# HerreraKrachTeichmann/NJODE

Measured on AMD Instinct MI355X. Metric: paths/sec (training step) on 20k Black-Scholes, 100 steps, higher is better.
Workload: dtype f32; 1 GPU; BlackScholes 20000 paths/GPU x 100 grid steps, every rank's paths as one batch, hidden_size=10, 3x(50,50) tanh nets, dropout 0.1, train step = plan+fwd+bwd+Adam; global_batch=20000, n_obs_rows=199470, euler_steps_per_batch=1820212, params=10071, parallelism=dp1

## Files before the change

njode_amd/csrc/njode_cfg.hip:

```cpp
#include <type_traits>

#include "njode_route.h"
#if NJ_PART >= 4
#include "njode_chain.h"
#include "njode_chain_seg.h"
#include "njode_chain_dw.h"
#endif

#define NJ_CAT_(a, b) a##b
#define NJ_CAT(a, b) NJ_CAT_(a, b)

namespace njode {

#ifndef NJ_RNN
#define NJ_RNN 0
#endif
using C = Cfg<NJ_D, NJ_H, NJ_DO, NJ_NH, NJ_W, NJ_ACT, (NJ_MASKED != 0), (NJ_CURT != 0),
              (NJ_RES != 0), (NJ_RNN != 0)>;

hipError_t NJ_CAT(njode_seg_forward_, NJ_ID)(const KArgs& a, const Route& r, hipStream_t st);
hipError_t NJ_CAT(njode_seg_backward_, NJ_ID)(const KArgs& a, const Route& r, hipStream_t st);
constexpr bool HAS_MFMA = C::NH == 2 && !C::MASKED && !C::RNN && C::DO <= 16 && C::W < 64;
constexpr bool HAS_MFMA_LOCK = C::NH == 2 && !C::RNN && C::W < 64 && C::H <= 64 && C::DO <= 64;
constexpr bool HAS_MFMA_SWEEP =
// ... 68 lines not shown
    }
    if constexpr (HAS_SPLIT) {
      const int nb = (int)gridDim.x - n_pack;
      drop_bits_tile_steps<C>(a, ((int)blockIdx.x - n_pack) * 4 + (threadIdx.x >> 6), nb * 4);
    }
  }
}

template <class CC> static void launch_pack_frags(const KArgs& a, hipStream_t st, bool bits = false) {
  if constexpr (HAS_MFMA) {
    using ES = typename EncS<CC>::type;
    using DS = typename DecS<CC>::type;
    const int n_pack = cdiv((2 * MF<CC>::NALL + ES::NALL + DS::NALL) * 64, 256);
    if (bits) {
      const long long work = a.seg_chain ? (long long)a.K * a.B / 64 + 1
                                         : (long long)cdiv(a.n_obs, 16) * cdiv(a.K > 0 ? a.K : 1, 8);
      const int nb = (int)(work / 4 + 1 < 1024 ? work / 4 + 1 : 1024);
      k_pack_all_bits<CC, ES, DS><<<n_pack + nb, 256, 0, st>>>(a, n_pack);
    } else {
      k_pack_all<CC, ES, DS><<<n_pack, 256, 0, st>>>(a.P, a.frag, a.frag2, a.frag_enc, a.frag_dec, a.dc.inv_keep,
                                                  a.plan_sync_zero);
    }
  }
}
template <class CC, bool DROP> static void launch_mfma_enc(const KArgs& a, const Route& r, hipStream_t st) {
  if constexpr (HAS_MFMA) {
    const int n_tiles = cdiv(a.n_obs + a.B, 16);
    k_encode_rows_mfma<CC, DROP><<<n_tiles < r.enc_blocks ? n_tiles : r.enc_blocks, 64, 0, st>>>(a);
  }
}
template <class CC> static void lock_pack_frags(const KArgs& a, hipStream_t st) {
  if constexpr (HAS_MFMA_LOCK) {
    using ES = typename EncS<CC>::type;
    using DS = typename DecS<CC>::type;
    k_pack_frags<CC><<<cdiv(MF<CC>::NALL * 64, 256), 256, 0, st>>>(a.P, a.frag);
    k_pack_net<typename CC::Enc, ES><<<cdiv(ES::NALL * 64, 256), 256, 0, st>>>(a.P + CC::OFF_ENC,
                                                                             a.frag_enc);
    k_pack_net<typename CC::Dec, DS><<<cdiv(DS::NALL * 64, 256), 256, 0, st>>>(a.P + CC::OFF_DEC,
                                                                             a.frag_dec);
  }
}
template <class CC, bool DROP> static void launch_mfma_jump(const KArgs& a, hipStream_t st) {
  if constexpr (HAS_MFMA) {
    const int n_tiles = cdiv(a.n_obs, 16);
    k_jump_rows_mfma<CC, DROP><<<n_tiles < 2048 ? n_tiles : 2048, 64, 0, st>>>(a);
  }
}
template <class CC, bool DROP> static void launch_ode_bwd_mfma(const KArgs& a, const Route& r, hipStream_t st) {
  if constexpr (HAS_MFMA) {
    if constexpr (HAS_SPLIT) {
      if (r.ode_split) {
        ProfScope ps("k_ode_bwd_mixed", st);
        if (r.tile_q_on) k_ode_bwd_mixed<CC, DROP, true><<<a.n_blocks_bwd, 256, 0, st>>>(a);
        else k_ode_bwd_mixed<CC, DROP, false><<<a.n_blocks_bwd, 256, 0, st>>>(a);
        return;
      }
    }
    ProfScope ps("k_ode_bwd_mfma", st);
    k_ode_bwd_mfma<CC, DROP><<<a.n_waves_ode / 4, 256, 0, st>>>(a);
  }
}
template <class CC, bool DROP> static void launch_jump_rows_bwd(const KArgs& a, hipStream_t st) {
  if constexpr (HAS_MFMA) {
    ProfScope ps("k_jump_rows_bwd_mfma", st);
    k_jump_rows_bwd_mfma<CC, DROP><<<a.n_waves_rows / 4, 256, 0, st>>>(a);
  }
}
template <class CC, bool DROP>
static void launch_mfma_rows_bwd(const KArgs& a, const Route& r, hipStream_t st) {
  if constexpr (HAS_MFMA) {
    if (r.defer_loss != 2) launch_jump_rows_bwd<CC, DROP>(a, st);
    if (r.seg_chain) NJ_CAT(njode_seg_chain_backward_, NJ_ID)(a, r, st);
    else launch_ode_bwd_mfma<CC, DROP>(a, r, st);
    if (!r.dw_enc_fused) {
      ProfScope ps("k_encode_rows_bwd_mfma", st);
      k_encode_rows_bwd_mfma<CC, DROP><<<a.n_waves_rows / 4, 256, 0, st>>>(a);
    }
  }
}
template <class CC, bool DROP, bool TAIL>
static void launch_mfma_fwd(const KArgs& a, const Route& r, hipStream_t st) {
  if constexpr (HAS_MFMA) {
    const int n_tiles = cdiv(TAIL ? a.B : a.n_obs, 16);
    if constexpr (HAS_SPLIT) {
      if (r.ode_split) {
        if constexpr (TAIL) {
          k_ode_fwd_split<CC, DROP, true><<<n_tiles < 1024 ? n_tiles : 1024, 256, 0, st>>>(a);
        }
        else if (a.plan_job) {
          const PlanJob job = *(const PlanJob*)a.plan_job;
          k_ode_fwd_mixed_plan<CC, DROP, false><<<a.n_blocks_fwd + job.P, 256, 0, st>>>(a, job);
        }
        else if (r.enc_fused) k_ode_fwd_mixed<CC, DROP, true><<<a.n_blocks_fwd, 256, 0, st>>>(a);
        else k_ode_fwd_mixed<CC, DROP, false><<<a.n_blocks_fwd, 256, 0, st>>>(a);
        return;
      }
    }
    k_ode_fwd_mfma<CC, DROP, TAIL><<<n_tiles < 4096 ? n_tiles : 4096, 64, 0, st>>>(a);
  }
}

hipError_t NJ_CAT(njode_lock_forward_, NJ_ID)(const KArgs& a, const Route& r, hipStream_t st);
hipError_t NJ_CAT(njode_lock_backward_, NJ_ID)(const KArgs& a, const Route& r, hipStream_t st);

#if NJ_PART == 0
template <bool DROP, bool TAIL, int ODE> static void launch_ode_fwd(const KArgs& a, const Route& r, hipStream_t st) {
// ... 348 lines not shown
```

njode_amd/csrc/njode_kernels.h:

```cpp
#pragma once
#include "njode_device.h"

namespace njode {

constexpr uint32_t NET_ODE = 0, NET_ENC = 1, NET_DEC = 2, NET_DEC_BJ = 3, NET_DEC_ROW = 4;
constexpr uint32_t TKEY_START = 0xffffffffu;

template <int D_, int H_, int DO_, int NH_, int W_, int ACT_, bool MASKED_, bool CURT_,
          bool RES_, bool RNN_ = false>
struct Cfg {
  static constexpr int D = D_, H = H_, DO = DO_, NH = NH_, W = (NH_ > 0 ? W_ : 1), ACT = ACT_;
  static constexpr bool MASKED = MASKED_, CURT = CURT_, RES = RES_, RNN = RNN_;
  static constexpr int ODE_IN = D + H + (CURT ? 3 : 2);
  static constexpr int ENC_IN = MASKED ? 2 * D : D;
  using Ode = NetL<ODE_IN, H, NH, W_>;
  using Enc = NetL<ENC_IN, H, NH, W_>;
  using Dec = NetL<H, DO, NH, W_>;
  static constexpr int OFF_ODE = 0, OFF_ENC = Ode::SIZE, OFF_DEC = Ode::SIZE + Enc::SIZE;
  static constexpr int OFF_GRU = OFF_DEC + Dec::SIZE;
  static constexpr int G_WIH = 0, G_WHH = 3 * H * D, G_BIH = G_WHH + 3 * H * H, G_BHH = G_BIH + 3 * H;
  static constexpr int GRU_SIZE = G_BHH + 3 * H;
  static constexpr int P = OFF_GRU + (RNN ? GRU_SIZE : 0);
  static_assert(!(RNN && MASKED), "the GRU jump is not defined for masked models");
  static constexpr int ENC_CASE = !RES ? 0 : (D <= H ? 1 : 2);
// ... 294 lines not shown
      r = a.order[jj];
      b = a.obs_idx[r];
      n = valid ? a.item_len[r] : 0;
      kbeg = a.item_kbeg[r];
      prev = a.item_prev[r];
    }
    const int pv = prev >= 0 ? prev : 0;
    const float tprev = a.n_obs > 0 ? a.time_f32[a.t_of_row[pv]] : 0.0f;
    tau = prev >= 0 ? tprev : 0.0f;
    const float* xp = prev >= 0 ? a.X + (size_t)pv * C::D : a.start_X + (size_t)b * C::D;
#pragma unroll
    for (int i = 0; i < C::D; ++i) tx[i] = tanh_f(xp[i]);
  }
  NJ_DEV const float* h0(const KArgs& a) const {
    return prev >= 0 ? a.h0row + (size_t)prev * C::H : a.h0start + (size_t)b * C::H;
  }
  static constexpr int PACKF = 4 + 4 * ((1 + C::D + 3) / 4);
  NJ_DEV void store_pack(float* pack, int j) const {
    typedef float v4 __attribute__((ext_vector_type(4)));
    float* p = pack + (size_t)j * PACKF;
    const v4 head = {__int_as_float(r), __int_as_float(n), __int_as_float(kbeg), __int_as_float(b)};
    *(v4*)p = head;
#pragma unroll
    for (int q = 0; q < (PACKF - 4) / 4; ++q) {
      v4 v;
#pragma unroll
      for (int e = 0; e < 4; ++e) {
        const int i = 4 * q + e;
        v[e] = i == 0 ? tau : (i <= C::D ? tx[i - 1 < C::D ? (i > 0 ? i - 1 : 0) : 0] : 0.0f);
      }
      *(v4*)(p + 4 + 4 * q) = v;
    }
  }
  NJ_DEV void load_pack(const float* pack, int j, bool valid) {
    typedef float v4 __attribute__((ext_vector_type(4)));
    const float* p = pack + (size_t)j * PACKF;
    const v4 head = *(const v4*)p;
    r = __float_as_int(head[0]);
    n = valid ? __float_as_int(head[1]) : 0;
    kbeg = __float_as_int(head[2]);
    b = __float_as_int(head[3]);
    prev = -1;
#pragma unroll
    for (int q = 0; q < (PACKF - 4) / 4; ++q) {
      const v4 v = *(const v4*)(p + 4 + 4 * q);
#pragma unroll
      for (int e = 0; e < 4; ++e) {
        const int i = 4 * q + e;
        if (i == 0) tau = v[e];
        else if (i <= C::D) tx[i - 1 < C::D ? i - 1 : 0] = v[e];
      }
    }
  }
};

template <class C, bool DROP, bool TAIL, bool WLDS>
__global__ void __launch_bounds__(WLDS ? 256 : 64) k_ode_fwd_items(KArgs a) {
  const bool SAVE = !TAIL && a.save_traj != 0;
  constexpr int NT = WLDS ? 256 : 64;
  using NL = typename C::Ode;
  __shared__ __attribute__((aligned(16))) float wl[WLDS ? NL::SIZE : 4];
  if constexpr (WLDS) {
    for (int i = threadIdx.x; i < NL::SIZE; i += NT) wl[i] = a.P[C::OFF_ODE + i];
    __syncthreads();
  }
  const int n_items = TAIL ? a.B : a.n_obs;
  const int j = blockIdx.x * NT + threadIdx.x;
  const bool valid = j < n_items;
  Item<C> it;
  it.template load<TAIL>(a, j, valid);
  float h[C::H];
  load_vec(it.h0(a), h);
  const int nmax = wave_max(it.n);
  float* const trash = a.trash + threadIdx.x * C::H;
  for (int s = 0; s < nmax; ++s) {
    const bool active = s < it.n;
    const int k = active ? it.kbeg + s : 0;
    if (SAVE) {
      float* dst = active ? a.traj + (size_t)(a.base_s[s] + j) * C::H : trash;
      store_vec(dst, h);
    }
    const float dt = active ? a.step_dt[k] : 0.0f, t = a.step_t[k];
    float in0[C::ODE_IN], a1[C::W], a2[C::W], f[C::H];
    ode_input<C>(it.tx, h, it.tau, t, in0);
    Masks<C, DROP> mk;
    mk.draw(a, a.gid0 + it.b, (uint32_t)k, NET_ODE);
    if constexpr (WLDS)
      net_fwd<NL, C::ACT, DROP>((lcp)wl, in0, f, a1, a2, mk.m1, mk.m2, a.dc.inv_keep);
    else
      net_fwd<NL, C::ACT, DROP>(as_cfp(a.P) + C::OFF_ODE, in0, f, a1, a2, mk.m1, mk.m2,
                                a.dc.inv_keep);
#pragma unroll
    for (int i = 0; i < C::H; ++i) h[i] = fmaf(dt, f[i], h[i]);
  }
  float* out = TAIL ? a.hT + (size_t)it.b * C::H : a.h_end + (size_t)it.r * C::H;
  store_vec(valid ? out : trash, h);
}

template <class C, bool DROP>
__global__ void __launch_bounds__(64) k_jump_rows(KArgs a) {
  const int r = blockIdx.x * 64 + threadIdx.x;
  if (r >= a.n_obs) return;
  const int b = a.obs_idx[r];
  const uint32_t tkey = (uint32_t)a.k_jump[a.t_of_row[r]];
  const cfp Pd = as_cfp(a.P) + C::OFF_DEC;
  float h[C::H], th[C::H], a1[C::W], a2[C::W], y[C::DO], ybj[C::DO], x[C::D], mask[C::D];
// ... 318 lines not shown
```

njode_amd/csrc/njode_mfma_split.h:

```cpp
#pragma once
#include "njode_mfma.h"
#include "njode_ode2.h"
#include "njode_plan.h"

namespace njode {

template <class C, bool TWO = (C::NH == 2)> struct SplitOk { static constexpr bool value = false; };
template <class C> struct SplitOk<C, true> {
  static constexpr bool value = MF<C>::MT1 == 4 && MF<C>::MTH == 1 && !C::MASKED && !C::RNN;
};

constexpr int XROWS = 64;
constexpr int XFLOATS = XROWS * IMG_STRIDE;
constexpr int TROWS = 16;
constexpr int TFLOATS = TROWS * IMG_STRIDE;

template <class C, bool BWD> struct SplitFrags {
  using M = MF<C>;
  float A1[M::Q0], A2[M::Q1], A3[4];
  float B3[BWD ? M::QH : 1], B2[BWD ? M::QW : 1], B1[BWD ? 4 : 1];
  NJ_DEV void load(const float* frag, int w, int lane) {
#pragma unroll
    for (int q = 0; q < M::Q0; ++q) A1[q] = frag[(M::F1 + w * M::Q0 + q) * 64 + lane];
#pragma unroll
// ... 201 lines not shown
    s += PR[(3 * NQ + r) * 64 + lane];
    out[r] = s;
  }
}

template <class C> struct OdeFwdSplitLds { static constexpr int FLOATS = XFLOATS + 4 * MF<C>::QH * 64; };
template <class C, bool DROP, bool TAIL, bool SAVE>
NJ_DEV void ode_fwd_split(const KArgs& a, lfp lds_raw, int worker, int n_workers, int tile0, int tile1) {
  static_assert(!(TAIL && SAVE), "tail items are never checkpointed");
  using M = MF<C>;
  lfp X1 = lds_raw, PR = X1 + XFLOATS;
  const int lane = threadIdx.x & 63, g = lane >> 4, c = lane & 15;
  const int w = __builtin_amdgcn_readfirstlane(threadIdx.x >> 6);
  for (int i = threadIdx.x; i < XFLOATS; i += 256) lds_raw[i] = 0.0f;
  SplitFrags<C, false> F;
  F.load(a.frag, w, lane);
  In0Const<C> K0;
  K0.init(g);
  __syncthreads();
  const bool bits_ahead = DROP && !TAIL && a.dbits_ready != 0;

  const int n_items = TAIL ? a.B : a.n_obs;
  const int n_tiles = tile1 - tile0;
  float* const trash = a.trash + lane * C::H;
  for (int round = 0; round * n_workers < n_tiles; ++round) {
    const int rel = snake_tile(round, worker, n_workers);
    if (rel >= n_tiles) continue;
    const int tile = tile0 + rel;
    const int j = tile * 16 + c;
    const bool valid = j < n_items;
    Item<C> it;
    it.template load<TAIL>(a, j, valid);
    const float* h0 = it.h0(a);
    float h[M::QH];
#pragma unroll
    for (int q = 0; q < M::QH; ++q) {
      const int u = 4 * q + g;
      h[q] = u < C::H ? h0[u < C::H ? u : 0] : 0.0f;
    }
    const int nmax = uniform(wave_max(it.n));
    float dt_r = 0.0f, t_r = 0.0f;
    uint32_t kb_r = 0;
    long long b16_n = 0;
    if (nmax > 0) {
      const int k0 = it.n > 0 ? it.kbeg : 0;
      dt_r = a.step_dt[k0];
      t_r = a.step_t[k0];
      b16_n = (SAVE || bits_ahead) ? sload_ll(a.base16_s, 0) : 0;
      if (bits_ahead) kb_r = a.dbits[(size_t)(b16_n / 16 + tile) * 64 + lane];
    }
    if constexpr (SAVE) {
      if (a.item_pack) {
        if (w == 0 && g == 0) it.store_pack(a.item_pack, j);
        const long long bl = sload_ll(a.base16_s, nmax > 0 ? nmax - 1 : 0);
        if (threadIdx.x == 0) a.tile_last[tile] = bl;
      }
    }
    vm_drain();
    for (int s = 0; s < nmax; ++s) {
      const bool active = s < it.n;
      const int k = active ? it.kbeg + s : 0;
      const float dt = active ? dt_r : 0.0f, t = t_r;
      const uint32_t kb = kb_r;
      const long long b16 = b16_n;
      {
        const int sn = s + 1 < nmax ? s + 1 : s;
        const int kn = sn < it.n ? it.kbeg + sn : 0;
        dt_r = a.step_dt[kn];
        t_r = a.step_t[kn];
        if (SAVE || bits_ahead) b16_n = sload_ll(a.base16_s, sn);
        if (bits_ahead) kb_r = a.dbits[(size_t)(b16_n / 16 + tile) * 64 + lane];
      }
      float b0[M::Q0], a1l[4], a2l[4], a1u[4], a2u[4];
      in0_fill_c<C, 0>(b0, h, it.tx, it.tau, t - it.tau, g, K0);
      uint32_t k1 = 0, k2 = 0;
      if constexpr (DROP) {
        if (bits_ahead) {
          k1 = (kb >> (4 * w)) & 15u;
          k2 = (kb >> (16 + 4 * w)) & 15u;
        } else {
          split_keep_bits<C, DROP>(a, it.b, k, g, w, k1, k2);
        }
      }
      split_hidden_layers<C, DROP, false>(F, X1, b0, a1l, a2l, a1u, a2u, k1, k2, a.dc.inv_keep, g, c, w);
      if constexpr (SAVE) split_rec_store<C>(rec_block<C>(a.act, b16, tile), a.trash, lane, w, a1u, a2u, h);
      f32x4 part = {0.f, 0.f, 0.f, 0.f};
#pragma unroll
      for (int r = 0; r < 4; ++r)
        if (4 * w + r < M::Q1) part = mfma4(F.A3[r], a2l[r], part);
      float f[M::QH];
      split_reduce<M::QH>(PR, part, f, lane, w);
#pragma unroll
      for (int q = 0; q < M::QH; ++q) h[q] = fmaf(dt, f[q], h[q]);
    }
    if (w == 0) {
      float* out = valid ? (TAIL ? a.hT + (size_t)it.b * C::H : a.h_end + (size_t)it.r * C::H) : trash;
#pragma unroll
      for (int q = 0; q < M::QH; ++q) {
        const int u = 4 * q + g;
        float* dst = u < C::H ? out + u : trash;
        *dst = h[q];
      }
    }
  }
}

template <class C> struct OdeBwdSplitLds {
// ... 366 lines not shown
template <class C, bool DROP, bool TAIL>
__global__ void __launch_bounds__(256, 2) k_ode_fwd_split(KArgs a) {
  __shared__ __attribute__((aligned(16))) float lds_raw[OdeFwdSplitLds<C>::FLOATS];
  const int n_items = TAIL ? a.B : a.n_obs;
  ode_fwd_split<C, DROP, TAIL, false>(a, (lfp)lds_raw, blockIdx.x, gridDim.x, 0, (n_items + 15) / 16);
}

template <class C, bool ENC, bool PLAN> struct OdeFwdMixedLds {
  static constexpr int OWN = OdeFwdSplitLds<C>::FLOATS + (ENC ? EncFwdLds<C>::FLOATS : 0);
  static constexpr int FLOATS = (PLAN && PLAN_LDS_INTS > OWN) ? PLAN_LDS_INTS : OWN;
};
template <class C, bool DROP, bool ENC, bool PLAN>
__device__ __forceinline__ void ode_fwd_mixed_body(const KArgs& a, lfp lds_raw, int bid, int nblocks) {
  const int n_tiles = (a.n_obs + 15) / 16, ns = a.n_split_fwd;
  const int T = (int)a.base_s[a.K + 2];
  const bool save = a.save_traj != 0;
  if (save && bid == 0 && threadIdx.x == 0) { a.tile_q[0] = 0; a.tile_q[1] = 0; a.tile_q[2] = 0; }
  if (bid < ns) {
    if (save) ode_fwd_split<C, DROP, false, true>(a, lds_raw, bid, ns, 0, T);
    else ode_fwd_split<C, DROP, false, false>(a, lds_raw, bid, ns, 0, T);
  } else {
    const int wave = (bid - ns) * 4 + uniform(threadIdx.x >> 6);
    const int nw = (nblocks - ns) * 4;
    if constexpr (ENC) {
      lfp enc_img = lds_raw + OdeFwdSplitLds<C>::FLOATS;
      EncFwdLds<C>::stage(enc_img, a.frag_enc, threadIdx.x, 256);
      __syncthreads();
      if (save) ode2_fwd_single<C, DROP, false, true, true>(a, threadIdx.x & 63, wave, nw, T, n_tiles, enc_img);
      else ode2_fwd_single<C, DROP, false, false, true>(a, threadIdx.x & 63, wave, nw, T, n_tiles, enc_img);
    } else {
      if (save) ode2_fwd_single<C, DROP, false, true>(a, threadIdx.x & 63, wave, nw, T, n_tiles);
      else ode2_fwd_single<C, DROP, false, false>(a, threadIdx.x & 63, wave, nw, T, n_tiles);
    }
  }
}
template <class C, bool DROP, bool ENC = false>
__global__ void __launch_bounds__(256, 2) k_ode_fwd_mixed(KArgs a) {
  __shared__ __attribute__((aligned(16))) float lds_raw[OdeFwdMixedLds<C, ENC, false>::FLOATS];
  ode_fwd_mixed_body<C, DROP, ENC, false>(a, (lfp)lds_raw, blockIdx.x, gridDim.x);
}
template <class C, bool DROP, bool ENC = false>
__global__ void __launch_bounds__(256, 2) k_ode_fwd_mixed_plan(KArgs a, PlanJob job) {
  __shared__ __attribute__((aligned(16))) float lds_raw[OdeFwdMixedLds<C, ENC, true>::FLOATS];
  if ((int)blockIdx.x < job.P) {
    plan_grid_body(job, blockIdx.x, (int*)lds_raw);
    return;
  }
  ode_fwd_mixed_body<C, DROP, ENC, true>(a, (lfp)lds_raw, (int)blockIdx.x - job.P, (int)gridDim.x - job.P);
}
template <class C> struct OdeBwdMixedLds {
  static constexpr int A = OdeBwdActLds<C>::FLOATS, B = OdeBwdSplitLds<C>::FLOATS;
  static constexpr int FLOATS = A > B ? A : B;
};
template <class C, bool DROP, bool QUEUE = false>
__global__ void __launch_bounds__(256, 2) k_ode_bwd_mixed(KArgs a) {
  __shared__ __attribute__((aligned(16))) float lds_raw[OdeBwdMixedLds<C>::FLOATS];
  const int n_tiles = (a.n_obs + 15) / 16, ns = a.n_split_blocks;
  const int T = (int)a.base_s[a.K + 1];
#ifdef NJ_BWD_STAMPS
  BWD_STAMP(0, wall_clock64());
  BWD_STAMP(6, (unsigned long long)__builtin_amdgcn_s_getreg((31 << 11) | 4 ) |
                   ((unsigned long long)__builtin_amdgcn_s_getreg((31 << 11) | 20 ) << 32));
  BWD_STAMP(7, (unsigned long long)((int)blockIdx.x < ns ? 1 : 0) | ((unsigned long long)T << 8) |
                   ((unsigned long long)gridDim.x << 32));
#endif
  if constexpr (QUEUE) {
    if ((int)blockIdx.x < ns) {
      ode3_bwd_split<C, DROP, true>(a, (lfp)lds_raw, blockIdx.x, ns, 0, T, blockIdx.x, n_tiles);
    } else {
      const int wave = ((int)blockIdx.x - ns) * 4 + uniform(threadIdx.x >> 6);
      ode3_bwd_single<C, DROP, true>(a, (lfp)lds_raw, wave, ((int)gridDim.x - ns) * 4, T, n_tiles, blockIdx.x);
    }
    queue_block_done(a.tile_q, gridDim.x);
  } else {
    if ((int)blockIdx.x < ns) {
      ode3_bwd_split<C, DROP>(a, (lfp)lds_raw, blockIdx.x, ns, 0, T, blockIdx.x);
    } else {
      const int wave = ((int)blockIdx.x - ns) * 4 + uniform(threadIdx.x >> 6);
      ode3_bwd_single<C, DROP>(a, (lfp)lds_raw, wave, ((int)gridDim.x - ns) * 4, T, n_tiles, blockIdx.x);
    }
  }
}

}
```

njode_amd/csrc/njode_ode2.h:

```cpp
#pragma once
#include "njode_mfma.h"
#include "njode_mfma_rows.h"

namespace njode {

constexpr float TANH_PRESCALE = 2.8853900817779268f;

template <class C> struct Ode2Scale {
  static constexpr float S = C::ACT == ACT_TANH ? TANH_PRESCALE : 1.0f;
};

template <class C> NJ_DEV float ode_frag_value(const float* __restrict__ P, int idx, float S, float ik) {
  using M = MF<C>;
  const int f = idx >> 6, l = idx & 63, g = l >> 4, c = l & 15;
  const float* Po = P + C::OFF_ODE;
  using NL = typename C::Ode;
  const float *W1 = Po + NL::woff(0), *b1 = Po + NL::boff(0), *W2 = Po + NL::woff(1),
              *b2 = Po + NL::boff(1), *W3 = Po + NL::woff(2), *b3 = Po + NL::boff(2);
  float v = 0.0f;
  if (f < M::F2) {
    const int mt = (f - M::F1) / M::Q0, q = (f - M::F1) % M::Q0;
    const int uo = row_unit(mt, c), ui = 4 * q + g;
    if (uo < M::W) v = S * (ui < M::IN0 ? W1[uo * M::IN0 + M::col0(ui)] : (ui == M::IN0 ? b1[uo] : 0.0f));
  } else if (f < M::F3) {
// ... 322 lines not shown
    const float v = out[q / 4][q % 4] + enc_residual<C>(xp, u < C::H ? u : 0);
    h[q] = u < C::H ? v : 0.0f;
    float* dst = u < C::H ? dstrow + u : trash;
    *dst = v;
  }
}

template <class C, bool DROP, bool TAIL, bool SAVE, bool ENC = false>
NJ_DEV void ode2_fwd_single(const KArgs& a, int lane, int wave, int n_waves, int tile0, int tile1,
                            lfp enc_img = nullptr) {
  static_assert(!(TAIL && SAVE), "tail items are never checkpointed");
  static_assert(!(TAIL && ENC), "tails read the stored state after their last observation");
  using M = MF<C>;
  const int g = lane >> 4, c = lane & 15;
  Ode2FwdFrags<C> F;
  F.load(a.frag2, lane);
  In0Const<C> K0;
  K0.init(g);

  const int n_items = TAIL ? a.B : a.n_obs;
  const int n_tiles = tile1 - tile0;
  float* const trash = a.trash + lane * C::H;
  for (int round = 0; round * n_waves < n_tiles; ++round) {
    const int rel = snake_tile(round, wave, n_waves);
    if (rel >= n_tiles) continue;
    const int tile = tile0 + rel;
    const int j = tile * 16 + c;
    const bool valid = j < n_items;
    Item<C> it;
    it.template load<TAIL>(a, j, valid);
    float h[M::QH];
    if constexpr (ENC) {
      ode2_item_start<C, DROP>(a, it, valid, enc_img, lane, h);
    } else {
      const float* h0 = it.h0(a);
#pragma unroll
      for (int q = 0; q < M::QH; ++q) {
        const int u = 4 * q + g;
        h[q] = u < C::H ? h0[u < C::H ? u : 0] : 0.0f;
      }
    }
    const int nmax = uniform(wave_max(it.n));
    float dt_r = 0.0f, t_r = 0.0f;
    long long b16_n = 0;
    if (nmax > 0) {
      const int k0 = it.n > 0 ? it.kbeg : 0;
      dt_r = a.step_dt[k0];
      t_r = a.step_t[k0];
      b16_n = SAVE ? sload_ll(a.base16_s, 0) : 0;
    }
    if constexpr (SAVE) {
      if (a.item_pack) {
        if (g == 0) it.store_pack(a.item_pack, j);
        const long long bl = sload_ll(a.base16_s, nmax > 0 ? nmax - 1 : 0);
        if (lane == 0) a.tile_last[tile] = bl;
      }
    }
    vm_drain();
    for (int s = 0; s < nmax; ++s) {
      const bool active = s < it.n;
      const int k = active ? it.kbeg + s : 0;
      const float dt = active ? dt_r : 0.0f, t = t_r;
      const long long b16 = b16_n;
      {
        const int sn = s + 1 < nmax ? s + 1 : s;
        const int kn = sn < it.n ? it.kbeg + sn : 0;
        dt_r = a.step_dt[kn];
        t_r = a.step_t[kn];
        if constexpr (SAVE) b16_n = sload_ll(a.base16_s, sn);
      }
      float b0[M::Q0];
      in0_fill_c<C, 0>(b0, h, it.tx, it.tau, t - it.tau, g, K0);
      uint32_t st = 0;
      if constexpr (DROP) {
        const unsigned long long gid = a.gid0 + it.b;
        st = drop_state(a.dc, (uint32_t)gid, (uint32_t)(gid >> 32) + 0x5bd1e995u * (g + 1),
                        (uint32_t)k, NET_ODE);
      }
      float a1[M::Q1], a2[M::Q1];
      hidden_layer2<C, DROP, M::Q0>(F.A1, b0, a1, st, a.dc.thr16, g);
      float* blk = nullptr;
      if constexpr (SAVE) {
        blk = rec_block<C>(a.act, b16, tile);
        rec_store_B<C>(blk, lane, a1);
      }
      hidden_layer2<C, DROP, M::Q1>(F.A2, a1, a2, st, a.dc.thr16, g);
      if constexpr (SAVE) rec_store_A<C>(blk, lane, a2, h);
      f32x4 f[M::MTH];
      out_layer2<C>(F.A3, a2, f);
#pragma unroll
      for (int q = 0; q < M::QH; ++q) h[q] = fmaf(dt, f[q / 4][q % 4], h[q]);
    }
    float* out = valid ? (TAIL ? a.hT + (size_t)it.b * C::H : a.h_end + (size_t)it.r * C::H) : trash;
#pragma unroll
    for (int q = 0; q < M::QH; ++q) {
      const int u = 4 * q + g;
      float* dst = u < C::H ? out + u : trash;
      *dst = h[q];
    }
  }
}



template <class C> struct OdeLdsFragsT {
  using M = MF<C>;
  static constexpr int NVEC = M::NALL - M::NFWD;
// ... 124 lines not shown
    for (int r = 0; r < 4; ++r) {
      const int uo = 16 * mt + 4 * g + r;
      if (uo < M::W) {
#pragma unroll
        for (int nt = 0; nt < NT0; ++nt) {
          const int ui = 16 * nt + c;
          if (ui < M::IN0) W1[uo * M::IN0 + M::col0(ui)] = G1[mt][nt][r];
          else if (ui == M::IN0) b1[uo] = G1[mt][nt][r];
        }
      }
    }
#pragma unroll
  for (int mt = 0; mt < M::MTH; ++mt)
#pragma unroll
    for (int r = 0; r < 4; ++r) {
      const int uo = 16 * mt + 4 * g + r;
      if (uo < C::H) {
#pragma unroll
        for (int nt = 0; nt < NT1; ++nt) {
          const int ui = 16 * nt + c;
          if (ui < M::W) W3[uo * M::W + ui] = ik * G3[mt][nt][r];
          else if (ui == M::W) b3[uo] = G3[mt][nt][r];
        }
      }
    }
}

NJ_DEV int queue_pop_issue(int* q) {
  int t = 0;
  if ((threadIdx.x & 63) == 0) t = atomicAdd(q, 1);
  return t;
}
NJ_DEV int queue_value(int raw) { return __builtin_amdgcn_readfirstlane(raw); }
NJ_DEV void queue_block_done(int* tile_q, int n_blocks) {
  __syncthreads();
  if (threadIdx.x == 0) {
    __threadfence();
    if (atomicAdd(tile_q + 2, 1) == n_blocks - 1) {
      tile_q[0] = 0;
      tile_q[1] = 0;
      tile_q[2] = 0;
      __threadfence();
    }
  }
}
#ifdef NJ_BWD_STAMPS
__device__ unsigned long long g_bwd_stamps[8192 * 16];
#define BWD_STAMP(slot, val) \
  do { if ((threadIdx.x & 63) == 0) g_bwd_stamps[(size_t)(blockIdx.x * 4 + (threadIdx.x >> 6)) * 16 + (slot)] = (val); } while (0)
#else
#define BWD_STAMP(slot, val) do {} while (0)
#endif

template <class C, bool DROP, bool QUEUE = false>
NJ_DEV void ode3_bwd_single(const KArgs& a, lfp lds_raw, int wave, int n_waves, int tile0, int tile1,
                            int slab_row) {
  using M = MF<C>;
  using NL = typename C::Ode;
  using FR = OdeLdsFragsT<C>;
  constexpr int NT1 = (M::W + 1 + 15) / 16;
  constexpr int NT0 = (M::IN0 + 1 + 15) / 16;
  const int lane = threadIdx.x & 63, wv = threadIdx.x >> 6, g = lane >> 4, c = lane & 15;
  using IL = BwdIL;
  lfp img_d = lds_raw + wv * 2 * IL::FLOATS, img_a = img_d + IL::FLOATS;
  lfp fimg = lds_raw + 4 * 2 * IL::FLOATS;
  FR::stage(fimg, a.frag2, threadIdx.x, 256);
  for (int i = threadIdx.x; i < 4 * 2 * IL::FLOATS; i += 256) lds_raw[i] = 0.0f;
  __syncthreads();
  FR F;
  F.init(fimg, lane);
  In0Const<C> K0;
  K0.init(g);

  using E2 = OdeG2<C>;
  constexpr int ET = E2::ER ? E2::ET : -1, ER = E2::ER;
  const int de = edge_lane(lane) - lane;
  f32x4 G3[M::MTH][NT1], G2[E2::MT][E2::NT], GM[2], GN[2], G1[M::MT1][NT0];
  const f32x4 zero4 = {0.f, 0.f, 0.f, 0.f};
  GM[0] = GM[1] = GN[0] = GN[1] = zero4;
#pragma unroll
  for (int i = 0; i < M::MTH; ++i)
#pragma unroll
    for (int n = 0; n < NT1; ++n) G3[i][n] = zero4;
#pragma unroll
  for (int i = 0; i < E2::MT; ++i)
#pragma unroll
    for (int n = 0; n < E2::NT; ++n) G2[i][n] = zero4;
#pragma unroll
  for (int i = 0; i < M::MT1; ++i) {
#pragma unroll
    for (int n = 0; n < NT0; ++n) G1[i][n] = zero4;
  }
  float* const trash = a.trash + threadIdx.x * C::H;
  const int n_tiles = tile1 - tile0;
  BWD_STAMP(1, wall_clock64());
  int q_raw = 0;
  int q_rel = wave;
  int n_done = 0, n_steps_done = 0;
#ifdef NJ_BWD_STAMPS
  unsigned long long t_pro = 0, t_loop = 0, t_pop = 0;
#endif
  for (int round = 0; QUEUE ? q_rel < n_tiles : round * n_waves < n_tiles; ++round) {
#ifdef NJ_BWD_STAMPS
    const unsigned long long tt0 = wall_clock64();
#endif
    int rel;
    if constexpr (QUEUE) {
      rel = q_rel;
    } else {
      rel = snake_tile(round, wave, n_waves);
      if (rel >= n_tiles) continue;
    }
    const int tile = tile0 + rel;
    const int j = tile * 16 + c;
    const bool valid = j < a.n_obs;
    Item<C> it;
    long long b16_last = 0;
    const bool packed = a.item_pack != nullptr;
    if (packed) {
      b16_last = sload_ll(a.tile_last, tile);
      it.load_pack(a.item_pack, j, valid);
    } else {
      it.template load<false>(a, j, valid);
    }
    float lam[M::QH];
#pragma unroll
    for (int q = 0; q < M::QH; ++q) {
      const int u = 4 * q + g;
      const float v = a.lam_end[(size_t)it.r * C::H + (u < C::H ? u : 0)];
      lam[q] = (valid && u < C::H) ? v : 0.0f;
    }
    const int nmax = BWD_ABL(64) ? 0 : uniform(wave_max(it.n));
    ++n_done;
    n_steps_done += nmax;
    auto load_sched = [&](int s, float& dtr, float& tr) {
      const int kk = s < it.n ? it.kbeg + s : 0;
      dtr = a.step_dt[kk];
      tr = a.step_t[kk];
    };
    float h[M::QH], a1[M::Q1], a2[M::Q1], dt_r = 0.0f, t_r = 0.0f;
#pragma unroll
    for (int q = 0; q < M::QH; ++q) h[q] = 0.0f;
#pragma unroll
    for (int q = 0; q < M::Q1; ++q) { a1[q] = 0.0f; a2[q] = 0.0f; }
    if (nmax > 0) {
      const float* blk = rec_block<C>(a.act, packed ? b16_last : sload_ll(a.base16_s, nmax - 1), tile);
      load_sched(nmax - 1, dt_r, t_r);
      rec_load_A<C>(blk, lane, a2, h);
      rec_load_B<C>(blk, lane, a1);
    }
#ifdef NJ_BWD_STAMPS
    vm_drain();
    const unsigned long long tt1 = wall_clock64();
    t_pro += tt1 - tt0;
#endif
    if constexpr (QUEUE) q_raw = queue_pop_issue(a.tile_q + 1);
    for (int s = nmax - 1; s >= 0; --s) {
      const float dt = s < it.n ? dt_r : 0.0f, t = t_r;
      const int sp = s > 0 ? s - 1 : 0;
      const float* blkp = rec_block<C>(a.act, sload_ll(a.base16_s, sp), tile);
      float b0[M::Q0];
      in0_fill_c<C, 0>(b0, h, it.tx, it.tau, t - it.tau, g, K0);
      if (!BWD_ABL(8)) load_sched(sp, dt_r, t_r);
      F.begin();

      float d3[M::QH];
#pragma unroll
      for (int q = 0; q < M::QH; ++q) d3[q] = dt * lam[q];
      if (!BWD_ABL(16)) {
        img_write<M::QH, IL>(img_d, d3, g, c);
        img_write<M::Q1, IL>(img_a, a2, g, c);
      }
      if (!BWD_ABL(4)) wave_lds_sync();
      if (!BWD_ABL(1)) dw_accumulate<M::MTH, NT1, IL>(img_d, img_a, G3, g, c);
      f32x4 acc[M::MT1];
#pragma unroll
      for (int mt = 0; mt < M::MT1; ++mt) acc[mt] = zero4;
      if (!BWD_ABL(2)) {
#pragma unroll
        for (int q = 0; q < M::QH; ++q)
#pragma unroll
          for (int mt = 0; mt < M::MT1; ++mt)
            acc[mt] = mt == ET ? mfma1(F.e3(q, de), d3[q], acc[mt]) : mfma4(F.b3(mt, q), d3[q], acc[mt]);
        if constexpr (ER != 0) acc[ET] = edge_tile<ER>(acc[ET], g);
      } else {
#pragma unroll
        for (int mt = 0; mt < M::MT1; ++mt) acc[mt][0] = d3[0];
      }
      float d2[M::QW];
#pragma unroll
      for (int q = 0; q < M::QW; ++q)
        d2[q] = acc[q / 4][q % 4] * (BWD_ABL(32) ? 1.0f : dact_stored<C::ACT, DROP>(a2[q]));
      if (!BWD_ABL(8)) rec_load_A<C>(blkp, lane, a2, h);
      if (!BWD_ABL(4)) wave_lds_sync();

      if (!BWD_ABL(16)) {
        img_write<M::QW, IL>(img_d, d2, g, c);
        img_write<M::Q1, IL>(img_a, a1, g, c);
      }
      if (!BWD_ABL(4)) wave_lds_sync();
      if (!BWD_ABL(1)) {
        if constexpr (ER != 0) dw_accumulate_edge<E2::MT, IL>(img_d, img_a, G2, GM, GN, lane, g, c);
        else dw_accumulate<E2::MT, E2::NT, IL>(img_d, img_a, G2, g, c);
      }
#pragma unroll
      for (int mt = 0; mt < M::MT1; ++mt) acc[mt] = zero4;
      if (!BWD_ABL(2)) {
#pragma unroll
        for (int q = 0; q < M::QW; ++q)
#pragma unroll
          for (int mt = 0; mt < M::MT1; ++mt)
            acc[mt] = mt == ET ? mfma1(F.e2(q, de), d2[q], acc[mt]) : mfma4(F.b2(mt, q), d2[q], acc[mt]);
        if constexpr (ER != 0) acc[ET] = edge_tile<ER>(acc[ET], g);
      } else {
#pragma unroll
        for (int mt = 0; mt < M::MT1; ++mt) acc[mt][0] = d2[mt];
      }
      float d1[M::QW];
#pragma unroll
      for (int q = 0; q < M::QW; ++q)
        d1[q] = acc[q / 4][q % 4] * (BWD_ABL(32) ? 1.0f : dact_stored<C::ACT, DROP>(a1[q]));
      if (!BWD_ABL(8)) rec_load_B<C>(blkp, lane, a1);
      if (!BWD_ABL(4)) wave_lds_sync();

      if (!BWD_ABL(16)) {
        img_write<M::QW, IL>(img_d, d1, g, c);
        img_write<M::Q0, IL>(img_a, b0, g, c);
      }
      if (!BWD_ABL(4)) wave_lds_sync();
      if (!BWD_ABL(1)) dw_accumulate<M::MT1, NT0, IL>(img_d, img_a, G1, g, c);
      f32x4 acch[M::MTH];
#pragma unroll
      for (int mt = 0; mt < M::MTH; ++mt) {
        f32x4 e = zero4, o = zero4;
        if (!BWD_ABL(2)) {
#pragma unroll
          for (int q = 0; q < M::QW; q += 2) {
            e = mfma4(F.b1(mt, q), d1[q], e);
            if (q + 1 < M::QW) o = mfma4(F.b1(mt, q + 1), d1[q + 1], o);
          }
        } else {
          e[0] = d1[0];
        }
        acch[mt] = e + o;
      }
#pragma unroll
      for (int q = 0; q < M::QH; ++q) {
        const float th = b0[q];
        const float dth = (4 * q + g) < C::H ? 1.0f - th * th : 0.0f;
        lam[q] = fmaf(acch[q / 4][q % 4], dth, lam[q]);
      }
      if (!BWD_ABL(4)) wave_lds_sync();
    }
#ifdef NJ_BWD_STAMPS
    t_loop += wall_clock64() - tt1;
#endif
    float* out = valid ? a.lam_start + (size_t)it.r * C::H : trash;
#pragma unroll
    for (int q = 0; q < M::QH; ++q) {
      const int u = 4 * q + g;
      float* dst = u < C::H ? out + u : trash;
      *dst = lam[q];
    }
    if constexpr (QUEUE) {
#ifdef NJ_BWD_STAMPS
      const unsigned long long tq0 = wall_clock64();
#endif
      q_rel = n_waves + queue_value(q_raw);
#ifdef NJ_BWD_STAMPS
      t_pop += wall_clock64() - tq0;
#endif
    }
  }

#ifdef NJ_BWD_STAMPS
  BWD_STAMP(8, t_pro);
  BWD_STAMP(9, t_loop);
  BWD_STAMP(10, t_pop);
#endif
  BWD_STAMP(2, wall_clock64());
  BWD_STAMP(4, (unsigned long long)n_done);
  BWD_STAMP(5, (unsigned long long)n_steps_done);
  (void)n_done; (void)n_steps_done; (void)q_rel;
  if (BWD_ABL(128)) return;
  ode3_flush<C, DROP>(a, lds_raw, G3, G2, GM, GN, G1, slab_row);
  BWD_STAMP(3, wall_clock64());
}


}
```

Measured before the change: 23.14 million paths/s.

## Chain backward ODE tiles so each wave prefetches its next tile during the last step

Adds a CHAIN variant of the split backward ODE kernel, used when packed item records exist. On the final backward step of a tile, the wave already loads the next tile's recorded activations, item pack and schedule, so the next tile starts without a cold prologue. The tile_last sentinel becomes -1 for empty tiles so the chain can tell whether a record exists. This aims to hide per-tile prologue latency, at the cost of more live registers, a per-step item reload and extra control complexity.

```diff
diff --git a/njode_amd/csrc/njode_cfg.hip b/njode_amd/csrc/njode_cfg.hip
--- a/njode_amd/csrc/njode_cfg.hip
+++ b/njode_amd/csrc/njode_cfg.hip
@@ -144,6 +144,7 @@
       if (r.ode_split) {
         ProfScope ps("k_ode_bwd_mixed", st);
         if (r.tile_q_on) k_ode_bwd_mixed<CC, DROP, true><<<a.n_blocks_bwd, 256, 0, st>>>(a);
+        else if (a.item_pack) k_ode_bwd_mixed<CC, DROP, false, true><<<a.n_blocks_bwd, 256, 0, st>>>(a);
         else k_ode_bwd_mixed<CC, DROP, false><<<a.n_blocks_bwd, 256, 0, st>>>(a);
         return;
       }
diff --git a/njode_amd/csrc/njode_kernels.h b/njode_amd/csrc/njode_kernels.h
--- a/njode_amd/csrc/njode_kernels.h
+++ b/njode_amd/csrc/njode_kernels.h
@@ -370,6 +370,35 @@
       }
     }
   }
+  NJ_DEV void reload_pack(const float* pack, int j) {
+    typedef float v2 __attribute__((ext_vector_type(2)));
+    typedef float v3 __attribute__((ext_vector_type(3)));
+    typedef float v4 __attribute__((ext_vector_type(4)));
+    const float* p = pack + (size_t)j * PACKF;
+    const v3 head = *(const v3*)p;
+    r = __float_as_int(head[0]);
+    n = __float_as_int(head[1]);
+    kbeg = __float_as_int(head[2]);
+    float f[4 * ((1 + C::D + 3) / 4)];
+    constexpr int NQ = (1 + C::D) / 4, REM = (1 + C::D) % 4;
+#pragma unroll
+    for (int q = 0; q < NQ; ++q) {
+      const v4 v = *(const v4*)(p + 4 + 4 * q);
+      f[4 * q] = v[0]; f[4 * q + 1] = v[1]; f[4 * q + 2] = v[2]; f[4 * q + 3] = v[3];
+    }
+    if constexpr (REM == 3) {
+      const v3 v = *(const v3*)(p + 4 + 4 * NQ);
+      f[4 * NQ] = v[0]; f[4 * NQ + 1] = v[1]; f[4 * NQ + 2] = v[2];
+    } else if constexpr (REM == 2) {
+      const v2 v = *(const v2*)(p + 4 + 4 * NQ);
+      f[4 * NQ] = v[0]; f[4 * NQ + 1] = v[1];
+    } else if constexpr (REM == 1) {
+      f[4 * NQ] = p[4 + 4 * NQ];
+    }
+    tau = f[0];
+#pragma unroll
+    for (int i = 0; i < C::D; ++i) tx[i] = f[1 + i];
+  }
 };
 
 template <class C, bool DROP, bool TAIL, bool WLDS>
diff --git a/njode_amd/csrc/njode_mfma_split.h b/njode_amd/csrc/njode_mfma_split.h
--- a/njode_amd/csrc/njode_mfma_split.h
+++ b/njode_amd/csrc/njode_mfma_split.h
@@ -277,7 +277,7 @@
     if constexpr (SAVE) {
       if (a.item_pack) {
         if (w == 0 && g == 0) it.store_pack(a.item_pack, j);
-        const long long bl = sload_ll(a.base16_s, nmax > 0 ? nmax - 1 : 0);
+        const long long bl = nmax > 0 ? sload_ll(a.base16_s, nmax - 1) : -1;
         if (threadIdx.x == 0) a.tile_last[tile] = bl;
       }
     }
@@ -750,7 +750,7 @@
   static constexpr int A = OdeBwdActLds<C>::FLOATS, B = OdeBwdSplitLds<C>::FLOATS;
   static constexpr int FLOATS = A > B ? A : B;
 };
-template <class C, bool DROP, bool QUEUE = false>
+template <class C, bool DROP, bool QUEUE = false, bool CHAIN = false>
 __global__ void __launch_bounds__(256, 2) k_ode_bwd_mixed(KArgs a) {
   __shared__ __attribute__((aligned(16))) float lds_raw[OdeBwdMixedLds<C>::FLOATS];
   const int n_tiles = (a.n_obs + 15) / 16, ns = a.n_split_blocks;
@@ -775,9 +775,9 @@
       ode3_bwd_split<C, DROP>(a, (lfp)lds_raw, blockIdx.x, ns, 0, T, blockIdx.x);
     } else {
       const int wave = ((int)blockIdx.x - ns) * 4 + uniform(threadIdx.x >> 6);
-      ode3_bwd_single<C, DROP>(a, (lfp)lds_raw, wave, ((int)gridDim.x - ns) * 4, T, n_tiles, blockIdx.x);
-    }
-  }
-}
-
-}
+      ode3_bwd_single<C, DROP, false, CHAIN>(a, (lfp)lds_raw, wave, ((int)gridDim.x - ns) * 4, T, n_tiles, blockIdx.x);
+    }
+  }
+}
+
+}
diff --git a/njode_amd/csrc/njode_ode2.h b/njode_amd/csrc/njode_ode2.h
--- a/njode_amd/csrc/njode_ode2.h
+++ b/njode_amd/csrc/njode_ode2.h
@@ -398,7 +398,7 @@
     if constexpr (SAVE) {
       if (a.item_pack) {
         if (g == 0) it.store_pack(a.item_pack, j);
-        const long long bl = sload_ll(a.base16_s, nmax > 0 ? nmax - 1 : 0);
+        const long long bl = nmax > 0 ? sload_ll(a.base16_s, nmax - 1) : -1;
         if (lane == 0) a.tile_last[tile] = bl;
       }
     }
@@ -629,7 +629,7 @@
 #define BWD_STAMP(slot, val) do {} while (0)
 #endif
 
-template <class C, bool DROP, bool QUEUE = false>
+template <class C, bool DROP, bool QUEUE = false, bool CHAIN = false>
 NJ_DEV void ode3_bwd_single(const KArgs& a, lfp lds_raw, int wave, int n_waves, int tile0, int tile1,
                             int slab_row) {
   using M = MF<C>;
@@ -677,6 +677,15 @@
 #ifdef NJ_BWD_STAMPS
   unsigned long long t_pro = 0, t_loop = 0, t_pop = 0;
 #endif
+  static_assert(!(QUEUE && CHAIN), "the chained walk knows a worker's next tile from the static rounds");
+  Item<C> it;
+  float lam[M::QH], h[M::QH], a1[M::Q1], a2[M::Q1], dt_r = 0.0f, t_r = 0.0f;
+#pragma unroll
+  for (int q = 0; q < M::QH; ++q) { lam[q] = 0.0f; h[q] = 0.0f; }
+#pragma unroll
+  for (int q = 0; q < M::Q1; ++q) { a1[q] = 0.0f; a2[q] = 0.0f; }
+  bool pre = false;
+  int nmax_pre = 0;
   for (int round = 0; QUEUE ? q_rel < n_tiles : round * n_waves < n_tiles; ++round) {
 #ifdef NJ_BWD_STAMPS
     const unsigned long long tt0 = wall_clock64();
@@ -691,41 +700,53 @@
     const int tile = tile0 + rel;
     const int j = tile * 16 + c;
     const bool valid = j < a.n_obs;
-    Item<C> it;
-    long long b16_last = 0;
-    const bool packed = a.item_pack != nullptr;
-    if (packed) {
-      b16_last = sload_ll(a.tile_last, tile);
-      it.load_pack(a.item_pack, j, valid);
-    } else {
-      it.template load<false>(a, j, valid);
-    }
-    float lam[M::QH];
-#pragma unroll
-    for (int q = 0; q < M::QH; ++q) {
-      const int u = 4 * q + g;
-      const float v = a.lam_end[(size_t)it.r * C::H + (u < C::H ? u : 0)];
-      lam[q] = (valid && u < C::H) ? v : 0.0f;
-    }
-    const int nmax = BWD_ABL(64) ? 0 : uniform(wave_max(it.n));
-    ++n_done;
-    n_steps_done += nmax;
     auto load_sched = [&](int s, float& dtr, float& tr) {
       const int kk = s < it.n ? it.kbeg + s : 0;
       dtr = a.step_dt[kk];
       tr = a.step_t[kk];
     };
-    float h[M::QH], a1[M::Q1], a2[M::Q1], dt_r = 0.0f, t_r = 0.0f;
-#pragma unroll
-    for (int q = 0; q < M::QH; ++q) h[q] = 0.0f;
-#pragma unroll
-    for (int q = 0; q < M::Q1; ++q) { a1[q] = 0.0f; a2[q] = 0.0f; }
-    if (nmax > 0) {
-      const float* blk = rec_block<C>(a.act, packed ? b16_last : sload_ll(a.base16_s, nmax - 1), tile);
-      load_sched(nmax - 1, dt_r, t_r);
-      rec_load_A<C>(blk, lane, a2, h);
-      rec_load_B<C>(blk, lane, a1);
-    }
+    int nmax = nmax_pre;
+    if (!CHAIN || !pre) {
+      long long b16_last = 0;
+      const bool packed = CHAIN || a.item_pack != nullptr;
+      if (packed) {
+        b16_last = sload_ll(a.tile_last, tile);
+        it.load_pack(a.item_pack, j, valid);
+      } else {
+        it.template load<false>(a, j, valid);
+      }
+#pragma unroll
+      for (int q = 0; q < M::QH; ++q) {
+        const int u = 4 * q + g;
+        const float v = a.lam_end[(size_t)it.r * C::H + (u < C::H ? u : 0)];
+        lam[q] = (valid && u < C::H) ? v : 0.0f;
+      }
+      nmax = BWD_ABL(64) ? 0 : uniform(wave_max(it.n));
+      dt_r = 0.0f, t_r = 0.0f;
+#pragma unroll
+      for (int q = 0; q < M::QH; ++q) h[q] = 0.0f;
+#pragma unroll
+      for (int q = 0; q < M::Q1; ++q) { a1[q] = 0.0f; a2[q] = 0.0f; }
+      if (nmax > 0) {
+        const float* blk = rec_block<C>(a.act, packed ? b16_last : sload_ll(a.base16_s, nmax - 1), tile);
+        load_sched(nmax - 1, dt_r, t_r);
+        rec_load_A<C>(blk, lane, a2, h);
+        rec_load_B<C>(blk, lane, a1);
+      }
+    }
+    ++n_done;
+    n_steps_done += nmax;
+    int tile_n = tile;
+    bool has_next = false;
+    if constexpr (CHAIN) {
+      const int nrel = snake_tile(round + 1, wave, n_waves);
+      has_next = nmax > 0 && nrel < n_tiles;
+      tile_n = has_next ? tile0 + nrel : tile;
+    }
+    const long long b16_nl = CHAIN ? sload_ll(a.tile_last, tile_n) : -1;
+    const bool rec_next = has_next && b16_nl >= 0;
+    const int r_cur = it.r;
+    if constexpr (CHAIN) vm_drain();
 #ifdef NJ_BWD_STAMPS
     vm_drain();
     const unsigned long long tt1 = wall_clock64();
@@ -735,10 +756,15 @@
     for (int s = nmax - 1; s >= 0; --s) {
       const float dt = s < it.n ? dt_r : 0.0f, t = t_r;
       const int sp = s > 0 ? s - 1 : 0;
-      const float* blkp = rec_block<C>(a.act, sload_ll(a.base16_s, sp), tile);
+      const bool to_next = CHAIN && s == 0 && rec_next;
+      const long long b16_p = sload_ll(a.base16_s, sp);
+      const float* blkp = rec_block<C>(a.act, to_next ? b16_nl : b16_p, to_next ? tile_n : tile);
       float b0[M::Q0];
       in0_fill_c<C, 0>(b0, h, it.tx, it.tau, t - it.tau, g, K0);
       if (!BWD_ABL(8)) load_sched(sp, dt_r, t_r);
+      if constexpr (CHAIN) {
+        if (!BWD_ABL(8)) it.reload_pack(a.item_pack, (s == 0 ? tile_n : tile) * 16 + c);
+      }
       F.begin();
 
       float d3[M::QH];
@@ -830,15 +856,36 @@
       if (!BWD_ABL(4)) wave_lds_sync();
     }
 #ifdef NJ_BWD_STAMPS
-    t_loop += wall_clock64() - tt1;
-#endif
-    float* out = valid ? a.lam_start + (size_t)it.r * C::H : trash;
+    const unsigned long long tt2 = wall_clock64();
+    t_loop += tt2 - tt1;
+#endif
+    float lam_n[M::QH];
+    bool valid_n = false;
+    if (has_next) {
+      valid_n = tile_n * 16 + c < a.n_obs;
+#pragma unroll
+      for (int q = 0; q < M::QH; ++q) {
+        const int u = 4 * q + g;
+        lam_n[q] = a.lam_end[(size_t)it.r * C::H + (u < C::H ? u : 0)];
+      }
+      nmax_pre = uniform(wave_max(it.n));
+      if (nmax_pre > 0) load_sched(nmax_pre - 1, dt_r, t_r);
+    }
+    float* out = valid ? a.lam_start + (size_t)r_cur * C::H : trash;
 #pragma unroll
     for (int q = 0; q < M::QH; ++q) {
       const int u = 4 * q + g;
       float* dst = u < C::H ? out + u : trash;
       *dst = lam[q];
     }
+    if (has_next) {
+#pragma unroll
+      for (int q = 0; q < M::QH; ++q) lam[q] = (valid_n && 4 * q + g < C::H) ? lam_n[q] : 0.0f;
+    }
+    pre = has_next;
+#ifdef NJ_BWD_STAMPS
+    if constexpr (CHAIN) t_pro += wall_clock64() - tt2;
+#endif
     if constexpr (QUEUE) {
 #ifdef NJ_BWD_STAMPS
       const unsigned long long tq0 = wall_clock64();
```

Measured after the change: 23.24 million paths/s, median of 6. Within noise of the previous version (+0.4%).
